# Raspy-Py/VolumetricRenderer

Measured on AMD Instinct MI355X. Metric: Mray/s (= W*H*steps/s) at 1080p x 128 steps, higher is better.
Workload: dtype f32; 1 GPU; grid512: 512^3 RGBA8 grid, 1920x1080, 128 steps, RGBA8 out; width=1920, height=1080, max_steps=128, volume=512^3 RGBA8, camera=reference (TestMain.cpp:219-245), kernel=grid_col48_clamp_uG

## Files before the change

volumetricrenderer_amd/csrc/vr_ctx.h:

```cpp
#pragma once

#include <algorithm>
#include <cmath>
#include <cstdarg>
#include <cstdio>
#include <cstring>
#include <exception>
#include <new>
#include <stdexcept>
#include <string>
#include <vector>

#include "../../include/vr.h"
#include "vr_internal.h"

namespace vrapi {
using namespace vr;

extern thread_local std::string g_err;
vr_status fail(vr_status st, const char* fmt, ...);
vr_status caught_exception(const char* fn) noexcept;

#define HIP_TRY(expr)                                                                        \
    do {                                                                                     \
// ... 132 lines not shown
    bool region_exact = false;
    long long renders_since_build = 0;
    std::vector<float> sort_key;
    long long renders_since_sort = 0;
    int sort_reuse = 0;
    int lattice = 1;
    int inject_throw = 0;
    unsigned long long gen = 1;
    int launch_cache = 1;
    int empty_fill = 1;
    int frames_overlap = 0;
    int row_setup = 40, row_pow = 130;
    int row_first_pct = 100;
    struct Cached {
        bool valid = false;
        unsigned long long gen = 0;
        vr_target t{};
        hipStream_t stream = nullptr;
        GridFrame f;
    } lc[4];
    int lc_next = 0;
    long long lc_hits = 0;
    int pair_deal = 0;
    int frame_pairing = 2;
    long long pair_launches = 0;
    int frame_group = 4;
    long long group_launches = 0;
    int frame_quad = 1;
    long long quad_launches = 0;
    int quad_split = 1;
    long long quad_split_launches = 0;
    int quad_steps = 1;
    long long quad_steps_launches = 0;
    uint2* d_lat = nullptr;
    size_t lat_cap = 0;
    long long lat_key[3] = {0, 0, -1};
};

constexpr long long kMaxWorleyTableBytes = 32 << 10;

int auto_layout(int nx, int ny, int nz);
Ctx* as_ctx(void* p);
void free_volume(Ctx* c);
bool dims_ok(int nx, int ny, int nz);
int wanted_fast_layout(const Ctx* c);
vr_status ensure_fast_layout(Ctx* c, hipStream_t s);
vr_status install_volume(Ctx* c, const uint8_t* d_rgba, int nx, int ny, int nz, hipStream_t s);
vr_status resolve_uniform(Ctx* c);
vr_status ensure_blur(Ctx* c, size_t need);
vr_status release_blur(Ctx* c);
void tap_constants(const Ctx* c, float S[4][3], float T[4][3]);
bool clamp_is_exact(const Ctx* c, const float S[4][3], const float T[4][3]);
int band_rows_packed(int height, int band_rows, int band_stride, int band_first, int band_flip = 0);
vr_status make_plan(Ctx* c, MarchArgs* a, Plan* p);
bool frame_args(const Ctx* c, int width, int height, MarchArgs* a);
inline float acc_limit_of(float transmittance, float density, float step_size)
{
    return transmittance > 0.0f ? (float)(-std::log((double)transmittance) / ((double)density * (double)step_size))
                                : INFINITY;
}
void proc_args(const Ctx* c, MarchArgs* a);
void volume_args(const Ctx* c, const Plan& pl, MarchArgs* a);
const char* variant_name(const Plan& p);

struct TargetInfo {
    int format;
// ... 33 lines not shown
```

volumetricrenderer_amd/csrc/vr_internal.h:

```cpp
#pragma once
#include <hip/hip_runtime.h>
#include <stdint.h>
#include <stddef.h>
#include "../../include/vr.h"
#include "vr_dispatch.h"

namespace vr {

enum Layout : int {
    LAYOUT_PLANAR = 1,
    LAYOUT_BRICK5 = 2,
    LAYOUT_BRICK8 = 3,
    LAYOUT_BRICK16 = 4,
    LAYOUT_CORNER8 = 5,
    LAYOUT_BRICK4 = 6,
    LAYOUT_ZPAIR = 7,
    LAYOUT_BRICK448 = 8,
    LAYOUT_BRICK488 = 9,
    LAYOUT_BRICK4816 = 10,
    LAYOUT_BRICK41616 = 11,
    LAYOUT_BRICK4832 = 12,
    LAYOUT_BRICK4864 = 13,
    LAYOUT_CORNERH = 14,
    LAYOUT_COL48 = 15,
// ... 135 lines not shown
    void* out;
    long long pitch;
    int format;
    int empty_fill;
    int bands_in_place;
    unsigned long long* step_counter;
    ProcParams proc;
    int slab_cap;
};

template <int L>
constexpr size_t march_lds_bytes(const MarchArgs& a)
{
    if (L == LAYOUT_PLANAR || L == LAYOUT_CORNERH) return 0;
    return (size_t)(a.nx + a.ny + a.nz + 3) * sizeof(unsigned) * (L == LAYOUT_COL48Z ? 2 : 1);
}

constexpr bool has_u_kernels(int l)
{
    return l == LAYOUT_COL48 || l == LAYOUT_BRICK4832 || l == LAYOUT_CORNERH || l == LAYOUT_COL48Z;
}
constexpr int u_kernel_channel(bool early, bool zero_offsets, int umask)
{
    if (early || !zero_offsets) return -1;
    return umask == 1 ? 0 : umask == 2 ? 1 : umask == 4 ? 2 : umask == 8 ? 3 : -1;
}

constexpr bool quad_instance(int layout, bool early, bool zero_offsets, int umask)
{
    if (u_kernel_channel(early, zero_offsets, umask) >= 0) return true;
    return !(is_b4_family(layout) && !early && zero_offsets);
}

enum QuadMode : int { QUAD_NONE = 0, QUAD_FRAMES = 1, QUAD_SPLIT = 2, QUAD_STEPS = 3 };
constexpr bool quad_split_layout(int layout) { return layout == LAYOUT_COL48 || layout == LAYOUT_BRICK4832; }

template <bool EARLY>
__host__ __device__ inline float quad_round_accumulate(float acc, float t0, float t1, float t2, float t3, int base, int n,
                                                       float acc_limit, bool* stop)
{
    bool st = false;
    const float t[4] = {t0, t1, t2, t3};
    for (int j = 0; j < 4; ++j) {
        acc = base + j < n && !st ? acc + t[j] : acc;
        if (EARLY) st = acc > acc_limit;
    }
    *stop = st;
    return acc;
}

struct FrameArgs {
    float org[3], o[3], px[3], py[3];
    float r2[4], r3[4];
    int cam_mode;
    float cam[3];
    float tap_T[4][3];
    int empty_fill;
    void* out;
    unsigned long long* step_counter;
};
__host__ __device__ inline FrameArgs frame_part(const MarchArgs& a)
{
    FrameArgs f{};
    for (int i = 0; i < 3; ++i) { f.org[i] = a.org[i]; f.o[i] = a.o[i]; f.px[i] = a.px[i]; f.py[i] = a.py[i]; f.cam[i] = a.cam[i]; }
    for (int i = 0; i < 4; ++i) { f.r2[i] = a.r2[i]; f.r3[i] = a.r3[i]; }
    for (int t = 0; t < 4; ++t)
        for (int i = 0; i < 3; ++i) f.tap_T[t][i] = a.tap_T[t][i];
    f.cam_mode = a.cam_mode;
// ... 308 lines not shown
```

volumetricrenderer_amd/csrc/vr_march_kernels.h:

```cpp
#pragma once
#include "vr_march_common.h"
#include "vr_noise.h"

namespace vr {
namespace {

constexpr int kTile = 16;

__device__ __forceinline__ float lerp_(float a, float b, float t) { return fmaf(t, b - a, a); }
__device__ __forceinline__ f2 lerp2(f2 a, f2 b, f2 t) { return __builtin_elementwise_fma(t, b - a, a); }
__device__ __forceinline__ int clampi(int v, int lo, int hi) { return min(max(v, lo), hi); }

__device__ __forceinline__ int cvt_flr(float x)
{
    int r;
    asm("v_cvt_flr_i32_f32 %0, %1" : "=v"(r) : "v"(x));
    return r;
}
__device__ __forceinline__ float fract_(float x) { return __builtin_amdgcn_fractf(x); }

template <int K>
__device__ __forceinline__ float ubyte(unsigned v)
{
    float r;
// ... 244 lines not shown
        float t0, t1, t2, t3;
        if constexpr (LAYOUT != LAYOUT_PLANAR) {
            t0 = blend_u<UM, 0, LAYOUT>(fetch_u<UM, 0, LAYOUT, ZO>(a, f, pxy, pz), uv);
            t1 = blend_u<UM, 1, LAYOUT>(fetch_u<UM, 1, LAYOUT, ZO>(a, f, pxy, pz), uv);
            t2 = blend_u<UM, 2, LAYOUT>(fetch_u<UM, 2, LAYOUT, ZO>(a, f, pxy, pz), uv);
            t3 = blend_u<UM, 3, LAYOUT>(fetch_u<UM, 3, LAYOUT, ZO>(a, f, pxy, pz), uv);
        } else {
            t0 = tap<LAYOUT, WRAP>(a, f, 0, pxy, pz);
            t1 = tap<LAYOUT, WRAP>(a, f, 1, pxy, pz);
            t2 = tap<LAYOUT, WRAP>(a, f, 2, pxy, pz);
            t3 = tap<LAYOUT, WRAP>(a, f, 3, pxy, pz);
        }
        acc = acc + ((t0 * t1) * (t2 + t3)) * (LAYOUT == LAYOUT_CORNERH ? f.scale : a.scale);
        pxy = pxy + r.sxy;
        pz = pz + r.sz;
        if constexpr (EARLY) {
            if (acc > a.acc_limit) { ++i; break; }
        }
    }
    if (r.live) {
        const float at = acc * a.step_size;
        store_pixel(a, x, orow, r.n >= 0, 1.0f - spec_expf(a.density * fminf(-at, 0.0f)));
    }
    return r.n > 0 ? (unsigned)i : 0u;
}

template <int J>
__device__ __forceinline__ unsigned quad_lane(unsigned v)
{
    return (unsigned)__builtin_amdgcn_update_dpp(0, (int)v, J * 0x55, 0xf, 0xf, true);
}
template <int K>
__device__ __forceinline__ float ubyte_of(unsigned v) { return (float)((v >> (8 * K)) & 0xffu); }

constexpr unsigned kSplitZ = 32;

struct SliceRaw {
    unsigned s0, s1, off;
};
template <int UM, int T, bool ZO>
__device__ __forceinline__ SliceRaw split_fetch(const MarchArgs& a, const FastCtx& f, f2 pxy, float pz, unsigned zoff)
{
    if constexpr ((UM >> T) & 1) {
        return SliceRaw{};
    } else {
        const f2 Tt = ZO ? f2{0.5f, 0.5f} : f2{a.tap_T[T][0], a.tap_T[T][1]};
        const f2 gxy = __builtin_elementwise_fma(pxy, f2{a.tap_S[T][0], a.tap_S[T][1]}, Tt);
        const float gz = fmaf(pz, a.tap_S[T][2], ZO ? 0.5f : a.tap_T[T][2]);
        const unsigned off = f.tx[cvt_flr(gxy.x)] + f.ty[cvt_flr(gxy.y)] + f.tz[cvt_flr(gz)];
        const auto s = __builtin_amdgcn_raw_buffer_load_b64(f.rsrc[T], (off & ~3u) + zoff, 0, 0);
        return SliceRaw{s[0], s[1], off};
    }
}
__device__ __forceinline__ unsigned split_pack(const SliceRaw& r)
{
    const unsigned q0 = __builtin_amdgcn_alignbyte(r.s1, r.s0, r.off);
    const unsigned q1 = __builtin_amdgcn_alignbyte(r.s1, r.s1, r.off);
    return __builtin_amdgcn_perm(q1, q0, 0x05040100u);
}
template <int UM, int T, int H, bool ZO>
__device__ __forceinline__ float split_blend(const MarchArgs& a, unsigned pk, f2 pxy, float pz, const float* uv)
{
    if constexpr ((UM >> T) & 1) {
        return uv[T];
    } else {
        const f2 Tt = ZO ? f2{0.5f, 0.5f} : f2{a.tap_T[T][0], a.tap_T[T][1]};
        const f2 gxy = __builtin_elementwise_fma(pxy, f2{a.tap_S[T][0], a.tap_S[T][1]}, Tt);
        const float gz = fmaf(pz, a.tap_S[T][2], ZO ? 0.5f : a.tap_T[T][2]);
// ... 34 lines not shown
            const unsigned p0 = split_pack(c0), p1 = split_pack(c1), p2 = split_pack(c2), p3 = split_pack(c3);
            bool stop = false;
            {
                const float t0 = split_blend<UM, 0, 0, ZO>(a, p0, axy, az, uv), t1 = split_blend<UM, 1, 0, ZO>(a, p1, axy, az, uv);
                const float t2 = split_blend<UM, 2, 0, ZO>(a, p2, axy, az, uv), t3 = split_blend<UM, 3, 0, ZO>(a, p3, axy, az, uv);
                acc = acc + ((t0 * t1) * (t2 + t3)) * a.scale;
                if constexpr (EARLY) stop = acc > a.acc_limit;
            }
            __builtin_amdgcn_sched_barrier(0);
            {
                const float t0 = split_blend<UM, 0, 1, ZO>(a, p0, bxy, bz, uv), t1 = split_blend<UM, 1, 1, ZO>(a, p1, bxy, bz, uv);
                const float t2 = split_blend<UM, 2, 1, ZO>(a, p2, bxy, bz, uv), t3 = split_blend<UM, 3, 1, ZO>(a, p3, bxy, bz, uv);
                const float both = acc + ((t0 * t1) * (t2 + t3)) * a.scale;
                acc = i + 1 < r.n && !stop ? both : acc;
                if constexpr (EARLY) stop = acc > a.acc_limit;
            }
            i += 2;
            if (stop || i >= r.n) break;
            c0 = n0; c1 = n1; c2 = n2; c3 = n3;
            axy = cxy; az = cz;
            bxy = dxy; bz = dz;
        }
    }
    if (r.live) {
        const float at = acc * a.step_size;
        store_pixel(a, x, orow, r.n >= 0, 1.0f - spec_expf(a.density * fminf(-at, 0.0f)));
    }
}

struct StepRaw {
    unsigned s00, s01, s10, s11, off;
    float wx, wy, wz;
};
template <int UM, int T, bool ZO>
__device__ __forceinline__ StepRaw step_fetch(const MarchArgs& a, const FastCtx& f, f2 pxy, float pz)
{
    if constexpr ((UM >> T) & 1) {
        return StepRaw{};
    } else {
        const f2 Tt = ZO ? f2{0.5f, 0.5f} : f2{a.tap_T[T][0], a.tap_T[T][1]};
        const f2 gxy = __builtin_elementwise_fma(pxy, f2{a.tap_S[T][0], a.tap_S[T][1]}, Tt);
        const float gz = fmaf(pz, a.tap_S[T][2], ZO ? 0.5f : a.tap_T[T][2]);
        const unsigned off = f.tx[cvt_flr(gxy.x)] + f.ty[cvt_flr(gxy.y)] + f.tz[cvt_flr(gz)];
        const auto s0 = __builtin_amdgcn_raw_buffer_load_b64(f.rsrc[T], off & ~3u, 0, 0);
        const auto s1 = __builtin_amdgcn_raw_buffer_load_b64(f.rsrc[T], (off & ~3u) + kSplitZ, 0, 0);
        return StepRaw{s0[0], s0[1], s1[0], s1[1], off, fract_(gxy.x), fract_(gxy.y), fract_(gz)};
    }
}
__device__ __forceinline__ TapRaw step_tap(const StepRaw& r)
{
    return TapRaw{__builtin_amdgcn_alignbyte(r.s01, r.s00, r.off), __builtin_amdgcn_alignbyte(r.s01, r.s01, r.off),
                  __builtin_amdgcn_alignbyte(r.s11, r.s10, r.off), __builtin_amdgcn_alignbyte(r.s11, r.s11, r.off),
                  r.wx, r.wy, r.wz};
}
template <int J>
__device__ __forceinline__ float quad_lane_f(float v)
{
    return __builtin_bit_cast(float, quad_lane<J>(__builtin_bit_cast(unsigned, v)));
}
template <int LAYOUT, bool EARLY, bool ZO, int UM>
__device__ __forceinline__ void march_pixel_quad_steps(const MarchArgs& a, const FastCtx& f, int x, int orow, int fl)
{
    static_assert(quad_split_layout(LAYOUT), "built for the layouts of the split fetch");
    const Ray r = setup_ray(a, x, orow);
    float uv[4] = {};
    if constexpr (UM != 0)
        for (int t = 0; t < 4; ++t)
            if ((UM >> t) & 1) uv[t] = noise::in_vgpr(a.uval[t]);
    float acc = 0.0f;
    if (r.n > 0) {
        const auto own = [fl](auto p0, auto p1, auto p2, auto p3) { return fl & 2 ? (fl & 1 ? p3 : p2) : (fl & 1 ? p1 : p0); };
        f2 axy = r.pxy;
        float az = r.pz;
        f2 bxy = axy + r.sxy, cxy = bxy + r.sxy, dxy = cxy + r.sxy;
        float bz = az + r.sz, cz = bz + r.sz, dz = cz + r.sz;
        bool mine = fl < r.n;
        f2 qxy = mine ? own(axy, bxy, cxy, dxy) : axy;
        float qz = mine ? own(az, bz, cz, dz) : az;
        StepRaw c0 = step_fetch<UM, 0, ZO>(a, f, qxy, qz), c1 = step_fetch<UM, 1, ZO>(a, f, qxy, qz);
        StepRaw c2 = step_fetch<UM, 2, ZO>(a, f, qxy, qz), c3 = step_fetch<UM, 3, ZO>(a, f, qxy, qz);
        for (int base = 0;;) {
            const f2 exy = dxy + r.sxy, fxy = exy + r.sxy, gxy = fxy + r.sxy, hxy = gxy + r.sxy;
            const float ez = dz + r.sz, fz = ez + r.sz, gz = fz + r.sz, hz = gz + r.sz;
            mine = base + 4 + fl < r.n;
            qxy = mine ? own(exy, fxy, gxy, hxy) : axy;
            qz = mine ? own(ez, fz, gz, hz) : az;
            const StepRaw n0 = step_fetch<UM, 0, ZO>(a, f, qxy, qz), n1 = step_fetch<UM, 1, ZO>(a, f, qxy, qz);
            const StepRaw n2 = step_fetch<UM, 2, ZO>(a, f, qxy, qz), n3 = step_fetch<UM, 3, ZO>(a, f, qxy, qz);
            const float t0 = blend_u<UM, 0, LAYOUT>(step_tap(c0), uv), t1 = blend_u<UM, 1, LAYOUT>(step_tap(c1), uv);
            const float t2 = blend_u<UM, 2, LAYOUT>(step_tap(c2), uv), t3 = blend_u<UM, 3, LAYOUT>(step_tap(c3), uv);
            const float term = ((t0 * t1) * (t2 + t3)) * a.scale;
            __builtin_amdgcn_sched_barrier(0);
            bool stop;
            acc = quad_round_accumulate<EARLY>(acc, quad_lane_f<0>(term), quad_lane_f<1>(term), quad_lane_f<2>(term),
                                               quad_lane_f<3>(term), base, r.n, a.acc_limit, &stop);
            base += 4;
            if (stop || base >= r.n) break;
            c0 = n0; c1 = n1; c2 = n2; c3 = n3;
            axy = exy; az = ez;
            dxy = hxy; dz = hz;
        }
    }
    if (r.live) {
        const float at = acc * a.step_size;
        store_pixel(a, x, orow, r.n >= 0, 1.0f - spec_expf(a.density * fminf(-at, 0.0f)));
    }
}

template <int LAYOUT>
__device__ __forceinline__ FastCtx fast_prologue(const MarchArgs& a, unsigned* lds)
{
    FastCtx f{};
    if constexpr (LAYOUT == LAYOUT_CORNERH) {
        for (int c = 0; c < 4; ++c)
            f.rsrc[c] = __builtin_amdgcn_make_buffer_rsrc((void*)(a.vol + (size_t)c * a.plane_stride), (short)0,
                                                          (int)a.plane_stride, 0x00020000);
        f.s1x16 = (float)(16 * a.geom.nbx);
        f.s2x16 = (float)(16 * a.geom.nbx) * (float)a.geom.nby;
        for (int c = 0; c < 4; ++c) {
            f.sz[c] = noise::in_vgpr(a.tap_S[c][2]);
            f.oz[c] = noise::in_vgpr(a.tap_T[c][2]);
        }
        f.scale = noise::in_vgpr(a.scale);
// ... 111 lines not shown
    if ((int)(blockIdx.x >> 3) * WGW >= count) return;
#ifdef VR_TIMELINE
    const unsigned long long t_begin = __builtin_amdgcn_s_memrealtime();
#endif
    const FastCtx f = fast_prologue<LAYOUT>(a, lds);
    const int lane = threadIdx.x & 63;
    unsigned long long steps = 0;
    for (int k = w; w < nwx && k < count; k += nwx) {
        const unsigned t = tiles[begin + k];
        const int tx = (int)(t & 0xffffu), ty = (int)(t >> 16);
        steps += march_pixel<LAYOUT, WRAP, EARLY, ZO, UM>(a, f, tx * 8 + lane_x<LAYOUT>(lane),
                                                          ty * 8 + lane_y<LAYOUT>(lane));
    }
#ifdef VR_TIMELINE
    timeline_record(t_begin, steps);
#endif
    if (a.step_counter) add_steps(a, steps);
}
template <int LAYOUT, int WRAP, bool EARLY, bool ZO, int WGW = kThreads / 64>
__global__ __launch_bounds__(64 * WGW) void march_regions(const MarchArgs a, const unsigned* __restrict__ tiles,
                                                         const int* __restrict__ hdr, int nwx)
{
    extern __shared__ __attribute__((aligned(16))) unsigned lds[];
    regions_body<LAYOUT, WRAP, EARLY, ZO, WGW, 0>(a, tiles, hdr, nwx, lds);
}
template <int LAYOUT, int WRAP, bool EARLY, bool ZO, int UM>
__global__ __launch_bounds__(kThreads) void march_regions_u(const MarchArgs a, const unsigned* __restrict__ tiles,
                                                           const int* __restrict__ hdr, int nwx)
{
    extern __shared__ __attribute__((aligned(16))) unsigned lds[];
    regions_body<LAYOUT, WRAP, EARLY, ZO, kThreads / 64, UM>(a, tiles, hdr, nwx, lds);
}

template <int LAYOUT, int WRAP, bool EARLY, bool ZO, int UM, int NF, bool QUAD = false, bool SPLIT = false, bool STEPS = false>
__device__ __forceinline__ void regions_frames_body(const FramesArgs<NF>& g, const unsigned* __restrict__ tiles,
                                                    const int* __restrict__ hdr, int nwx, int deal, unsigned* lds)
{
    static_assert(NF == 2 || NF == 4, "a 4-wave workgroup is 4 / NF entry waves x NF frames");
    static_assert(!QUAD || NF == 4, "a quad of lanes is four frames");
    static_assert(!SPLIT || QUAD, "the lanes of a quad split a fetch only where they hold one ray");
    static_assert(!STEPS || SPLIT, "the step rounds are a split launch's");
    const int xcd = blockIdx.x & 7, wg = (int)(blockIdx.x >> 3);
    const int wave = __builtin_amdgcn_readfirstlane((int)(threadIdx.x >> 6));
    int fr = wave, first = wg, w = wg;
    if constexpr (NF == 2) {
        fr = deal ? (wg & 1) : (wave & 1);
        first = deal ? (wg >> 1) * 4 : wg * 2;
        w = first + (deal ? wave : (wave >> 1));
    }
    const int begin = hdr[xcd], all = hdr[xcd + 1] - begin;
    const int marched = min(hdr[kRegionWork + xcd], all);
    MarchArgs a = g.c;
    set_frame(&a, g.fr[fr]);
    const int count = a.empty_fill ? marched : all;
    if (a.empty_fill) fill_empty_tiles(a, tiles, begin, count, all, w, nwx);
    bool every = g.fr[0].empty_fill;
    for (int k = 1; k < NF; ++k) every = every && g.fr[k].empty_fill;
    if (first >= (every ? marched : all)) return;
    FastCtx f = fast_prologue<LAYOUT>(g.c, lds);
    const int lane = threadIdx.x & 63;
    if constexpr (QUAD) {
        MarchArgs q = g.c;
        const int fl = lane & 3;
        void* out = g.fr[0].out;
        for (int k = 1; k < NF; ++k) out = fl == k ? g.fr[k].out : out;
        q.out = out;
        const int qx = (wave & 1) * 4 + ((lane >> 2) & 3), qy = (wave >> 1) * 4 + (lane >> 4);
        const int qcount = g.c.empty_fill ? marched : all;
        for (int k = wg; wg < nwx && k < qcount; k += nwx) {
            const unsigned t = tiles[begin + k];
            const int tx = (int)(t & 0xffffu), ty = (int)(t >> 16);
            if constexpr (STEPS) march_pixel_quad_steps<LAYOUT, EARLY, ZO, UM>(q, f, tx * 8 + qx, ty * 8 + qy, fl);
            else if constexpr (SPLIT) march_pixel_quad_split<LAYOUT, EARLY, ZO, UM>(q, f, tx * 8 + qx, ty * 8 + qy, fl);
            else (void)march_pixel<LAYOUT, WRAP, EARLY, ZO, UM>(q, f, tx * 8 + qx, ty * 8 + qy);
        }
        return;
    }
    if constexpr (LAYOUT == LAYOUT_CORNERH)
        for (int c = 0; c < 4; ++c) f.oz[c] = noise::in_vgpr(a.tap_T[c][2]);
    unsigned long long steps = 0;
    for (int k = w; w < nwx && k < count; k += nwx) {
        const unsigned t = tiles[begin + k];
        const int tx = (int)(t & 0xffffu), ty = (int)(t >> 16);
        steps += march_pixel<LAYOUT, WRAP, EARLY, ZO, UM>(a, f, tx * 8 + lane_x<LAYOUT>(lane),
                                                          ty * 8 + lane_y<LAYOUT>(lane));
    }
    if (a.step_counter) add_steps(a, steps);
}
#define VR_SPLIT_WAVES __attribute__((amdgpu_waves_per_eu(SPLIT && (!STEPS || ZO) ? 5 : 1)))
template <int LAYOUT, int WRAP, bool EARLY, bool ZO, int NF, bool QUAD = false, bool SPLIT = false, bool STEPS = false>
__global__ __launch_bounds__(kThreads) VR_SPLIT_WAVES void march_regions_frames(const FramesArgs<NF> g, const unsigned* __restrict__ tiles,
                                                                const int* __restrict__ hdr, int nwx, int deal)
{
    extern __shared__ __attribute__((aligned(16))) unsigned lds[];
    regions_frames_body<LAYOUT, WRAP, EARLY, ZO, 0, NF, QUAD, SPLIT, STEPS>(g, tiles, hdr, nwx, deal, lds);
}
template <int LAYOUT, int WRAP, bool EARLY, bool ZO, int UM, int NF, bool QUAD = false, bool SPLIT = false, bool STEPS = false>
__global__ __launch_bounds__(kThreads) VR_SPLIT_WAVES void march_regions_frames_u(const FramesArgs<NF> g, const unsigned* __restrict__ tiles,
                                                                  const int* __restrict__ hdr, int nwx, int deal)
{
    extern __shared__ __attribute__((aligned(16))) unsigned lds[];
    regions_frames_body<LAYOUT, WRAP, EARLY, ZO, UM, NF, QUAD, SPLIT, STEPS>(g, tiles, hdr, nwx, deal, lds);
}
#undef VR_SPLIT_WAVES


template <int LAYOUT, bool EARLY, bool ZO, int K, int UM = 0>
__device__ __forceinline__ unsigned march_pixel_split(const MarchArgs& a, const FastCtx& f, int x, int orow,
                                                      int k, int ray_lane)
{
    constexpr int R = 64 / K;
    const Ray r = setup_ray(a, x, orow);
    float uv[4] = {};
    if constexpr (UM != 0)
        for (int t = 0; t < 4; ++t)
            if ((UM >> t) & 1) uv[t] = noise::in_vgpr(a.uval[t]);
    const int n = r.n;
    f2 pxy = r.pxy;
    float pz = r.pz;
    for (int j = 0; j < k; ++j) { pxy = pxy + r.sxy; pz = pz + r.sz; }
    float acc = 0.0f;
    int i = 0;
    if (n > 0) {
        const bool mine0 = k < n;
        TapRaw c0 = fetch_u<UM, 0, LAYOUT, ZO>(a, f, mine0 ? pxy : r.pxy, mine0 ? pz : r.pz);
        TapRaw c1 = fetch_u<UM, 1, LAYOUT, ZO>(a, f, mine0 ? pxy : r.pxy, mine0 ? pz : r.pz);
        TapRaw c2 = fetch_u<UM, 2, LAYOUT, ZO>(a, f, mine0 ? pxy : r.pxy, mine0 ? pz : r.pz);
        TapRaw c3 = fetch_u<UM, 3, LAYOUT, ZO>(a, f, mine0 ? pxy : r.pxy, mine0 ? pz : r.pz);
        for (int base = 0; base < n; base += K) {
            for (int j = 0; j < K; ++j) { pxy = pxy + r.sxy; pz = pz + r.sz; }
            const bool mine = base + K + k < n;
            const f2 qxy = mine ? pxy : r.pxy;
            const float qz = mine ? pz : r.pz;
            const TapRaw n0 = fetch_u<UM, 0, LAYOUT, ZO>(a, f, qxy, qz), n1 = fetch_u<UM, 1, LAYOUT, ZO>(a, f, qxy, qz);
            const TapRaw n2 = fetch_u<UM, 2, LAYOUT, ZO>(a, f, qxy, qz), n3 = fetch_u<UM, 3, LAYOUT, ZO>(a, f, qxy, qz);
// ... 180 lines not shown
    if (sc.kind == SCHED_REGIONS) return regions(std::integral_constant<int, 4>{});
#if VR_EXPERIMENTS
    if (sc.kind == SCHED_XCDROWS) {
        const int groups = (((a.width + 7) >> 3) + 3) >> 2, rows8 = (a.out_rows + 7) >> 3;
        const dim3 grid(8 * ((rows8 + 7) / 8) * groups);
        return with_bool(early, [&](auto E) {
            hipLaunchKernelGGL((march_xcdrows<L, W, E>), grid, block, lds, s, a);
            return hipGetLastError();
        });
    }
    if (sc.kind == SCHED_QUEUE) {
        hipError_t e = hipMemsetAsync(sc.heads, 0, 32, s);
        if (e != hipSuccess) return e;
        const dim3 grid(256 * sc.waves_per_simd);
        return with_bool(early, [&](auto E) {
            hipLaunchKernelGGL((march_queue<L, W, E>), grid, block, lds, s, a, sc.heads);
            return hipGetLastError();
        });
    }
#endif
    const dim3 grid(a.num_blocks);
    return with_bool(early, [&](auto E) {
        hipLaunchKernelGGL((march_grid<L, W, E>), grid, block, lds, s, a);
        return hipGetLastError();
    });
}

template <int L, int W>
hipError_t launch_frames_l(const MarchArgs& a, const FrameArgs* fr, int nf, bool early, const Schedule& sc, int deal, int quad,
                           hipStream_t s)
{
    if (quad != QUAD_NONE && (nf != kGroupFrames || !quad_instance(L, early, a.zero_offsets != 0, a.umask)))
        return hipErrorInvalidValue;
    if ((quad == QUAD_SPLIT || quad == QUAD_STEPS) && !quad_split_layout(L)) return hipErrorInvalidValue;
    return with_value<2, kGroupFrames>(nf, [&](auto NF) { return with_value<QUAD_NONE, QUAD_FRAMES, QUAD_SPLIT, QUAD_STEPS>(quad, [&](auto QD) {
        constexpr bool Q = decltype(QD)::value != QUAD_NONE && decltype(NF)::value == kGroupFrames;
        constexpr bool ST = Q && decltype(QD)::value == QUAD_STEPS && quad_split_layout(L);
        constexpr bool SP = (Q && decltype(QD)::value == QUAD_SPLIT && quad_split_layout(L)) || ST;
        FramesArgs<NF> g;
        g.c = a;
        for (int k = 0; k < NF; ++k) g.fr[k] = fr[k];
        const size_t lds = march_lds_bytes<L>(a);
        const dim3 block(kThreads);
        static_assert(has_u_kernels(L), "every multi-frame layout has the _u kernels");
        static_assert(kThreads == 64 * 4, "a workgroup is 4 / NF entry waves x NF frames");
        const int nwx = sc.map.nwx;
        const int dl = NF == 4 ? 0 : deal;
        const dim3 grid((unsigned)(NF == 4 ? 8 * nwx : dl ? 16 * ((nwx + 3) / 4) : 8 * ((nwx + 1) / 2)));
        if (u_kernel_channel(early, a.zero_offsets, a.umask) >= 0)
            return with_value<1, 2, 4, 8>(a.umask, [&](auto U) {
                hipLaunchKernelGGL((march_regions_frames_u<L, W, false, true, U, NF, Q, SP, ST>), grid, block, lds, s, g, sc.tiles, sc.hdr, nwx, dl);
                return hipGetLastError();
            }, hipErrorInvalidValue);
        return with_bool(early, [&](auto E) { return with_bool(a.zero_offsets, [&](auto Z) {
            constexpr bool QG = Q && quad_instance(L, decltype(E)::value, decltype(Z)::value, 0);
            hipLaunchKernelGGL((march_regions_frames<L, W, E, Z, NF, QG, QG && SP, QG && ST>), grid, block, lds, s, g, sc.tiles, sc.hdr, nwx, dl);
            return hipGetLastError();
        }); });
    }, hipErrorInvalidValue); }, hipErrorInvalidValue);
}

}
}
```

volumetricrenderer_amd/csrc/vr_options.cpp:

```cpp
#include "vr_ctx.h"

using namespace vrapi;

extern "C" {

vr_status vr_set_layout_preference(void* p, int pref)
try {
    if (!p || pref < 0 || pref >= kNumLayouts) return fail(VR_ERR_INVALID, "vr_set_layout_preference: bad argument");
    if (pref > 0 && !layout_built(pref))
        return fail(VR_ERR_INVALID, "vr_set_layout_preference: layout %d is built only with VR_EXPERIMENTS "
                                    "(make EXPERIMENTS=1; measured slower, DESIGN.md sec. 4)", pref);
    Ctx* c = as_ctx(p);
    ++c->gen;
    HIP_TRY(hipSetDevice(c->device));
    c->layout_pref = pref;
    vr_status st = ensure_fast_layout(c, nullptr);
    if (st == VR_OK && hipDeviceSynchronize() != hipSuccess) return fail(VR_ERR_HIP, "vr_set_layout_preference: sync");
    return st;
} catch (...) {
    return caught_exception("vr_set_layout_preference");
}

vr_status vr_set_option(void* p, const char* name, int value)
try {
// ... 32 lines not shown
        if (value < 0 || value > 1) return fail(VR_ERR_INVALID, "vr_set_option: empty_fill is 0 or 1");
        c->empty_fill = value;
        ++c->gen;
        return VR_OK;
    }
    if (n == "frame_pairing") {
        if (value < 0 || value > 2) return fail(VR_ERR_INVALID, "vr_set_option: frame_pairing is 0, 1 or 2");
        c->frame_pairing = value;
        return VR_OK;
    }
    if (n == "frame_group") {
        if (value != 2 && value != 4) return fail(VR_ERR_INVALID, "vr_set_option: frame_group is 2 or 4");
        c->frame_group = value;
        return VR_OK;
    }
    if (n == "pair_deal") {
        if (value < 0 || value > 1) return fail(VR_ERR_INVALID, "vr_set_option: pair_deal is 0 or 1");
        c->pair_deal = value;
        return VR_OK;
    }
    if (n == "frame_quad") {
        if (value < 0 || value > 1) return fail(VR_ERR_INVALID, "vr_set_option: frame_quad is 0 or 1");
        c->frame_quad = value;
        return VR_OK;
    }
    if (n == "quad_split") {
        if (value < 0 || value > 1) return fail(VR_ERR_INVALID, "vr_set_option: quad_split is 0 or 1");
        c->quad_split = value;
        return VR_OK;
    }
    if (n == "quad_steps") {
        if (value < 0 || value > 1) return fail(VR_ERR_INVALID, "vr_set_option: quad_steps is 0 or 1");
        c->quad_steps = value;
        return VR_OK;
    }
    if (n == "inject_throw") {
        if (value < 0 || value > 2)
            return fail(VR_ERR_INVALID, "vr_set_option: inject_throw is 0, 1 (std::runtime_error) or 2 (std::bad_alloc)");
        c->inject_throw = value;
        return VR_OK;
    }
    if (n == "schedule") {
        if (value < -1 || value > 5)
            return fail(VR_ERR_INVALID, "vr_set_option: schedule is -1 (auto), 0 (static), 1 (queue), "
                                        "2 (strided), 3 (xcd rows), 4 (rings) or 5 (regions)");
        c->schedule = value;
        return VR_OK;
    }
    if (n == "waves_per_simd") {
        if (value < 1 || value > 8) return fail(VR_ERR_INVALID, "vr_set_option: waves_per_simd in [1, 8]");
        c->waves_per_simd = value;
        return VR_OK;
    }
    if (n == "tiles_per_wave") {
        if (value < 0 || value > 64)
            return fail(VR_ERR_INVALID, "vr_set_option: tiles_per_wave in [1, 64], or 0 for auto");
        c->tiles_per_wave = value;
        return VR_OK;
    }
    if (n == "split") {
        if (value != 0 && value != 1 && value != 2 && value != 4 && value != 8)
            return fail(VR_ERR_INVALID, "vr_set_option: split is 0 (auto), 1, 2, 4 or 8");
        c->split = value;
        return VR_OK;
    }
    if (n == "wedges") {
// ... 131 lines not shown
    if (n == "blur_scratch_kib") return (int)std::min<size_t>(c->blur_bytes / 1024, 0x7fffffff);
    if (n == "slab_cap") return c->slab_cap;
    if (n == "region_order") return c->region_order;
    if (n == "sort_reuse") return c->sort_reuse;
    if (n == "wg_waves") return c->wg_waves;
    if (n == "uniform_skip") return c->uniform_skip;
    if (n == "region_work_tiles")
        return c->region_cur >= 0 ? c->region[c->region_cur].nwork : -1;
    if (n == "region_empty_tiles") {
        poll_region_header(c);
        return c->region_cur >= 0 ? c->region[c->region_cur].nempty : -1;
    }
    if (n == "uniform_mask") {
        if (!c->d_planar || resolve_uniform(c) != VR_OK) return -1;
        return c->uniform_mask;
    }
    if (n == "supertile") return c->supertile;
    if (n == "launch_cache") return c->launch_cache;
    if (n == "empty_fill") return c->empty_fill;
    if (n == "frames_overlap") return c->frames_overlap;
    if (n == "row_setup") return c->row_setup;
    if (n == "row_pow") return c->row_pow;
    if (n == "row_first_pct") return c->row_first_pct;
    if (n == "frame_pairing") return c->frame_pairing;
    if (n == "pair_deal") return c->pair_deal;
    if (n == "frame_group") return c->frame_group;
    if (n == "group_launches") return (int)std::min<long long>(c->group_launches, 0x7fffffff);
    if (n == "pair_launches") return (int)std::min<long long>(c->pair_launches, 0x7fffffff);
    if (n == "frame_quad") return c->frame_quad;
    if (n == "quad_split") return c->quad_split;
    if (n == "quad_split_launches") return (int)std::min<long long>(c->quad_split_launches, 0x7fffffff);
    if (n == "quad_steps") return c->quad_steps;
    if (n == "quad_steps_launches") return (int)std::min<long long>(c->quad_steps_launches, 0x7fffffff);
    if (n == "quad_launches") return (int)std::min<long long>(c->quad_launches, 0x7fffffff);
    if (n == "launch_cache_hits") return (int)std::min<long long>(c->lc_hits, 0x7fffffff);
    if (n == "experiments") return VR_EXPERIMENTS;
    if (n == "region_interval") return c->region_interval;
    if (n == "region_gpu") return c->region_gpu;
    if (n == "region_gpu_builds") return (int)std::min<long long>(c->gpu_builds, 0x7fffffff);
    return -1;
} catch (...) {
    (void)caught_exception("vr_get_option");
    return -1;
}

const char* vr_kernel_variant(void* p)
try {
    if (!p) return "none";
    Ctx* c = as_ctx(p);
    if (c->proc.enabled) {
        if (c->schedule == SCHED_STATIC) return c->proc.shadow_steps > 0 ? "procedural_shadow_tiles" : "procedural_tiles";
        if (c->schedule == SCHED_RINGS) return c->proc.shadow_steps > 0 ? "procedural_shadow_rings" : "procedural_rings";
        return c->proc.shadow_steps > 0 ? "procedural_shadow" : "procedural";
    }
    if (!c->d_planar || !c->has_camera) return "none";
    if (resolve_uniform(c) != VR_OK) return "none";
    MarchArgs a{};
    Plan pl{};
    make_plan(c, &a, &pl);
    const int kind = c->schedule >= 0 ? c->schedule : SCHED_REGIONS;
    if (pl.layout == LAYOUT_COL48 && c->slab && kind == SCHED_REGIONS && c->split <= 1)
        return pl.early ? "grid_col48_slab_clamp_early" : "grid_col48_slab_clamp";
    const int um = c->uniform_skip ? c->uniform_mask : 0;
    int ch = -1;
    if (kind == SCHED_REGIONS && c->wg_waves == 4 && has_u_kernels(pl.layout))
        ch = u_kernel_channel(pl.early, a.zero_offsets, um);
// ... 23 lines not shown
```

volumetricrenderer_amd/csrc/vr_render.cpp:

```cpp
#include "vr_ctx.h"

namespace vrapi {

vr_status check_frame_state(const char* fn, const Ctx* c, const vr_target* t)
{
    if (!c->d_planar && !c->proc.enabled)
        return fail(VR_ERR_NO_VOLUME, "%s: no volume (vr_set_volume / vr_generate_volume)", fn);
    if (!c->has_camera) return fail(VR_ERR_NO_CAMERA, "%s: no shader data (vr_set_shader_data)", fn);
    if (t->width <= 0 || t->height <= 0) return fail(VR_ERR_INVALID, "%s: bad size %dx%d", fn, t->width, t->height);
    return VR_OK;
}

vr_status check_pixels(const char* fn, const vr_target* t, int format, size_t* pitch)
{
    if (!t->pixels) return fail(VR_ERR_INVALID, "%s: pixels is null", fn);
    const int bpp = format_bytes(format);
    *pitch = t->row_pitch ? t->row_pitch : (size_t)t->width * bpp;
    if (*pitch < (size_t)t->width * bpp || *pitch % bpp != 0 || ((uintptr_t)t->pixels % bpp) != 0)
        return fail(VR_ERR_INVALID, "%s: pitch/alignment (pitch %zu, bpp %d)", fn, *pitch, bpp);
    return VR_OK;
}

vr_status check_target(const char* fn, const Ctx* c, const vr_target* t, TargetInfo* ti)
{
// ... 270 lines not shown
    bool grouped = groupable;
    for (int k = 1; k < n && groupable; ++k) {
        if (osd) st = vr_set_shader_data(p, &osd[k], &gsd[k]);
        if (st == VR_OK) st = grid_frame_args(c, &t[k], ti, &f[k]);
        if (st != VR_OK) {
            const std::string msg = g_err;
            vr_status rs = frame0_alone();
            if (rs == VR_OK) rs = render_plain(p, t, 1, k, osd, gsd, stream);
            if (osd) (void)vr_set_shader_data(p, &osd[k], &gsd[k]);
            g_err = msg;
            return st;
        }
        grouped = grouped && f[k].kind == f[0].kind && pair_compatible(f[0], f[k]);
    }
    if (!grouped) {
        st = frame0_alone();
        return st == VR_OK ? render_plain(p, t, 1, n, osd, gsd, stream) : st;
    }
    const Ctx::RegionBuf& rb = c->region[c->region_cur];
    FrameArgs fr[VR_MAX_GROUP];
    bool every = f[0].a.empty_fill != 0;
    for (int k = 0; k < n; ++k) {
        if (k > 0) f[k].a.empty_fill = f[0].a.empty_fill && same_region_camera(f[0], f[k]) ? 1 : 0;
        every = every && f[k].a.empty_fill;
        fr[k] = frame_part(f[k].a);
    }
    Schedule sc = f[0].sc;
    if (f[0].a.empty_fill && !every) sc.map.nwx = std::max(1, rb.map.nwx);
    bool quad = c->frame_quad && frames_share_camera(fr, n) &&
                quad_instance(f[0].pl.layout, f[0].pl.early, f[0].a.zero_offsets != 0, f[0].a.umask);
    for (int k = 0; k < n; ++k) quad = quad && !fr[k].step_counter;
    const bool split = quad && c->quad_split && quad_split_layout(f[0].pl.layout);
    const bool steps = split && c->quad_steps;
    HIP_TRY(launch_march_frames(f[0].a, fr, n, f[0].pl.layout, f[0].pl.early, sc, c->pair_deal,
                                steps ? QUAD_STEPS : split ? QUAD_SPLIT : quad ? QUAD_FRAMES : QUAD_NONE, hs));
    c->quad_launches += quad;
    c->quad_split_launches += split;
    c->quad_steps_launches += steps;
    c->group_launches += n == VR_MAX_GROUP;
    c->pair_launches += n / 2;
    c->renders_since_build += n - 1;
    c->region_slot = f[0].slot;
    return note_region_render(c, hs);
}

}

extern "C" {

vr_status vr_render(void* p, const vr_target* t, void* stream)
try {
    if (!p || !t) return fail(VR_ERR_INVALID, "vr_render: null argument");
    Ctx* c = as_ctx(p);
    TargetInfo ti;
    if (const vr_status st = check_target("vr_render", c, t, &ti)) return st;
    honour_inject_throw(c);
    const hipStream_t hs = static_cast<hipStream_t>(stream);
    if (c->proc.enabled) return render_procedural_frame(c, t, ti, hs);
    const GridFrame* hit = nullptr;
    if (const vr_status st = cache_hit(c, t, hs, &hit)) return st;
    if (hit) return launch_frame(c, *hit, nullptr, 0, hs);
    GridFrame f;
    if (const vr_status st = grid_frame_args(c, t, ti, &f)) return st;
    if (f.kind == SCHED_REGIONS)
        if (const vr_status st = attach_regions(c, hs, &f)) return st;
    return launch_frame(c, f, t, c->gen, hs);
} catch (...) {
    return caught_exception("vr_render");
}

vr_status vr_render_sequence(void* p, const vr_target* t, int frames, const vr_object_shader_data* osd,
// ... 61 lines not shown
```

Baseline: 6.205 million Mray/s.

## Pair z-slice fetches across quad lanes with DPP exchange in step rounds

```diff
diff --git a/volumetricrenderer_amd/csrc/vr_ctx.h b/volumetricrenderer_amd/csrc/vr_ctx.h
--- a/volumetricrenderer_amd/csrc/vr_ctx.h
+++ b/volumetricrenderer_amd/csrc/vr_ctx.h
@@ -188,6 +188,8 @@
     long long quad_split_launches = 0;
     int quad_steps = 1;
     long long quad_steps_launches = 0;
+    int quad_pairs = 1;
+    long long quad_pairs_launches = 0;
     uint2* d_lat = nullptr;
     size_t lat_cap = 0;
     long long lat_key[3] = {0, 0, -1};
diff --git a/volumetricrenderer_amd/csrc/vr_internal.h b/volumetricrenderer_amd/csrc/vr_internal.h
--- a/volumetricrenderer_amd/csrc/vr_internal.h
+++ b/volumetricrenderer_amd/csrc/vr_internal.h
@@ -191,8 +191,25 @@
     return !(is_b4_family(layout) && !early && zero_offsets);
 }
 
-enum QuadMode : int { QUAD_NONE = 0, QUAD_FRAMES = 1, QUAD_SPLIT = 2, QUAD_STEPS = 3 };
+enum QuadMode : int { QUAD_NONE = 0, QUAD_FRAMES = 1, QUAD_SPLIT = 2, QUAD_STEPS = 3, QUAD_PAIRS = 4 };
 constexpr bool quad_split_layout(int layout) { return layout == LAYOUT_COL48 || layout == LAYOUT_BRICK4832; }
+constexpr unsigned kSplitZ = 32;
+
+constexpr __host__ __device__ int pair_load_step(int instr, int fl) { return 2 * instr + (fl >> 1); }
+constexpr __host__ __device__ int pair_load_slice(int fl) { return fl & 1; }
+constexpr __host__ __device__ int pair_owner_instr(int j) { return j >> 1; }
+constexpr __host__ __device__ int pair_owner_lane(int j, int z) { return 2 * (j & 1) + z; }
+constexpr __host__ __device__ int quad_perm_ctrl(int l0, int l1, int l2, int l3) { return l0 | l1 << 2 | l2 << 4 | l3 << 6; }
+constexpr __host__ __device__ int pair_load_ctrl(int instr)
+{
+    return quad_perm_ctrl(pair_load_step(instr, 0), pair_load_step(instr, 1), pair_load_step(instr, 2), pair_load_step(instr, 3));
+}
+constexpr __host__ __device__ int pair_owner_ctrl(int z)
+{
+    return quad_perm_ctrl(pair_owner_lane(0, z), pair_owner_lane(1, z), pair_owner_lane(2, z), pair_owner_lane(3, z));
+}
+static_assert(pair_load_ctrl(0) == 0x50 && pair_load_ctrl(1) == 0xfa, "quad_perm [0,0,1,1] and [2,2,3,3]");
+static_assert(pair_owner_ctrl(0) == 0x88 && pair_owner_ctrl(1) == 0xdd, "quad_perm [0,2,0,2] and [1,3,1,3]");
 
 template <bool EARLY>
 __host__ __device__ inline float quad_round_accumulate(float acc, float t0, float t1, float t2, float t3, int base, int n,
diff --git a/volumetricrenderer_amd/csrc/vr_march_kernels.h b/volumetricrenderer_amd/csrc/vr_march_kernels.h
--- a/volumetricrenderer_amd/csrc/vr_march_kernels.h
+++ b/volumetricrenderer_amd/csrc/vr_march_kernels.h
@@ -300,8 +300,6 @@
 }
 template <int K>
 __device__ __forceinline__ float ubyte_of(unsigned v) { return (float)((v >> (8 * K)) & 0xffu); }
-
-constexpr unsigned kSplitZ = 32;
 
 struct SliceRaw {
     unsigned s0, s1, off;
@@ -402,8 +400,18 @@
     unsigned s00, s01, s10, s11, off;
     float wx, wy, wz;
 };
-template <int UM, int T, bool ZO>
-__device__ __forceinline__ StepRaw step_fetch(const MarchArgs& a, const FastCtx& f, f2 pxy, float pz)
+template <int J>
+__device__ __forceinline__ float quad_lane_f(float v)
+{
+    return __builtin_bit_cast(float, quad_lane<J>(__builtin_bit_cast(unsigned, v)));
+}
+template <int CTRL>
+__device__ __forceinline__ unsigned quad_read(unsigned v)
+{
+    return (unsigned)__builtin_amdgcn_update_dpp(0, (int)v, CTRL, 0xf, 0xf, true);
+}
+template <int UM, int T, bool ZO, bool PAIRS = false>
+__device__ __forceinline__ StepRaw step_fetch(const MarchArgs& a, const FastCtx& f, f2 pxy, float pz, int fl = 0)
 {
     if constexpr ((UM >> T) & 1) {
         return StepRaw{};
@@ -412,9 +420,18 @@
         const f2 gxy = __builtin_elementwise_fma(pxy, f2{a.tap_S[T][0], a.tap_S[T][1]}, Tt);
         const float gz = fmaf(pz, a.tap_S[T][2], ZO ? 0.5f : a.tap_T[T][2]);
         const unsigned off = f.tx[cvt_flr(gxy.x)] + f.ty[cvt_flr(gxy.y)] + f.tz[cvt_flr(gz)];
-        const auto s0 = __builtin_amdgcn_raw_buffer_load_b64(f.rsrc[T], off & ~3u, 0, 0);
-        const auto s1 = __builtin_amdgcn_raw_buffer_load_b64(f.rsrc[T], (off & ~3u) + kSplitZ, 0, 0);
-        return StepRaw{s0[0], s0[1], s1[0], s1[1], off, fract_(gxy.x), fract_(gxy.y), fract_(gz)};
+        if constexpr (PAIRS) {
+            const unsigned zoff = (unsigned)pair_load_slice(fl) * kSplitZ;
+            const unsigned al = off & ~3u;
+            const auto sa = __builtin_amdgcn_raw_buffer_load_b64(f.rsrc[T], quad_read<pair_load_ctrl(0)>(al) + zoff, 0, 0);
+            const auto sb = __builtin_amdgcn_raw_buffer_load_b64(f.rsrc[T], quad_read<pair_load_ctrl(1)>(al) + zoff, 0, 0);
+            const unsigned sh = (quad_read<pair_load_ctrl(0)>(off) & 3u) | (quad_read<pair_load_ctrl(1)>(off) << 2);
+            return StepRaw{sa[0], sa[1], sb[0], sb[1], sh, fract_(gxy.x), fract_(gxy.y), fract_(gz)};
+        } else {
+            const auto s0 = __builtin_amdgcn_raw_buffer_load_b64(f.rsrc[T], off & ~3u, 0, 0);
+            const auto s1 = __builtin_amdgcn_raw_buffer_load_b64(f.rsrc[T], (off & ~3u) + kSplitZ, 0, 0);
+            return StepRaw{s0[0], s0[1], s1[0], s1[1], off, fract_(gxy.x), fract_(gxy.y), fract_(gz)};
+        }
     }
 }
 __device__ __forceinline__ TapRaw step_tap(const StepRaw& r)
@@ -423,12 +440,23 @@
                   __builtin_amdgcn_alignbyte(r.s11, r.s10, r.off), __builtin_amdgcn_alignbyte(r.s11, r.s11, r.off),
                   r.wx, r.wy, r.wz};
 }
-template <int J>
-__device__ __forceinline__ float quad_lane_f(float v)
-{
-    return __builtin_bit_cast(float, quad_lane<J>(__builtin_bit_cast(unsigned, v)));
-}
-template <int LAYOUT, bool EARLY, bool ZO, int UM>
+template <int UM, int T>
+__device__ __forceinline__ float pair_blend(const StepRaw& r, int fl, const float* uv)
+{
+    if constexpr ((UM >> T) & 1) {
+        return uv[T];
+    } else {
+        const unsigned pa = split_pack(SliceRaw{r.s00, r.s01, r.off}), pb = split_pack(SliceRaw{r.s10, r.s11, r.off >> 2});
+        const unsigned a0 = quad_read<pair_owner_ctrl(0)>(pa), b0 = quad_read<pair_owner_ctrl(0)>(pb);
+        const unsigned a1 = quad_read<pair_owner_ctrl(1)>(pa), b1 = quad_read<pair_owner_ctrl(1)>(pb);
+        const bool second = pair_owner_instr(fl) != 0;
+        const unsigned z0 = second ? b0 : a0, z1 = second ? b1 : a1;
+        return blend(f2{ubyte_of<0>(z0), ubyte_of<0>(z1)}, f2{ubyte_of<1>(z0), ubyte_of<1>(z1)},
+                     f2{ubyte_of<2>(z0), ubyte_of<2>(z1)}, f2{ubyte_of<3>(z0), ubyte_of<3>(z1)}, r.wx, r.wy, r.wz);
+    }
+}
+
+template <int LAYOUT, bool EARLY, bool ZO, int UM, bool PAIRS = false>
 __device__ __forceinline__ void march_pixel_quad_steps(const MarchArgs& a, const FastCtx& f, int x, int orow, int fl)
 {
     static_assert(quad_split_layout(LAYOUT), "built for the layouts of the split fetch");
@@ -447,18 +475,20 @@
         bool mine = fl < r.n;
         f2 qxy = mine ? own(axy, bxy, cxy, dxy) : axy;
         float qz = mine ? own(az, bz, cz, dz) : az;
-        StepRaw c0 = step_fetch<UM, 0, ZO>(a, f, qxy, qz), c1 = step_fetch<UM, 1, ZO>(a, f, qxy, qz);
-        StepRaw c2 = step_fetch<UM, 2, ZO>(a, f, qxy, qz), c3 = step_fetch<UM, 3, ZO>(a, f, qxy, qz);
+        StepRaw c0 = step_fetch<UM, 0, ZO, PAIRS>(a, f, qxy, qz, fl), c1 = step_fetch<UM, 1, ZO, PAIRS>(a, f, qxy, qz, fl);
+        StepRaw c2 = step_fetch<UM, 2, ZO, PAIRS>(a, f, qxy, qz, fl), c3 = step_fetch<UM, 3, ZO, PAIRS>(a, f, qxy, qz, fl);
         for (int base = 0;;) {
             const f2 exy = dxy + r.sxy, fxy = exy + r.sxy, gxy = fxy + r.sxy, hxy = gxy + r.sxy;
             const float ez = dz + r.sz, fz = ez + r.sz, gz = fz + r.sz, hz = gz + r.sz;
             mine = base + 4 + fl < r.n;
             qxy = mine ? own(exy, fxy, gxy, hxy) : axy;
             qz = mine ? own(ez, fz, gz, hz) : az;
-            const StepRaw n0 = step_fetch<UM, 0, ZO>(a, f, qxy, qz), n1 = step_fetch<UM, 1, ZO>(a, f, qxy, qz);
-            const StepRaw n2 = step_fetch<UM, 2, ZO>(a, f, qxy, qz), n3 = step_fetch<UM, 3, ZO>(a, f, qxy, qz);
-            const float t0 = blend_u<UM, 0, LAYOUT>(step_tap(c0), uv), t1 = blend_u<UM, 1, LAYOUT>(step_tap(c1), uv);
-            const float t2 = blend_u<UM, 2, LAYOUT>(step_tap(c2), uv), t3 = blend_u<UM, 3, LAYOUT>(step_tap(c3), uv);
+            const StepRaw n0 = step_fetch<UM, 0, ZO, PAIRS>(a, f, qxy, qz, fl), n1 = step_fetch<UM, 1, ZO, PAIRS>(a, f, qxy, qz, fl);
+            const StepRaw n2 = step_fetch<UM, 2, ZO, PAIRS>(a, f, qxy, qz, fl), n3 = step_fetch<UM, 3, ZO, PAIRS>(a, f, qxy, qz, fl);
+            const float t0 = PAIRS ? pair_blend<UM, 0>(c0, fl, uv) : blend_u<UM, 0, LAYOUT>(step_tap(c0), uv);
+            const float t1 = PAIRS ? pair_blend<UM, 1>(c1, fl, uv) : blend_u<UM, 1, LAYOUT>(step_tap(c1), uv);
+            const float t2 = PAIRS ? pair_blend<UM, 2>(c2, fl, uv) : blend_u<UM, 2, LAYOUT>(step_tap(c2), uv);
+            const float t3 = PAIRS ? pair_blend<UM, 3>(c3, fl, uv) : blend_u<UM, 3, LAYOUT>(step_tap(c3), uv);
             const float term = ((t0 * t1) * (t2 + t3)) * a.scale;
             __builtin_amdgcn_sched_barrier(0);
             bool stop;
@@ -636,7 +666,8 @@
     regions_body<LAYOUT, WRAP, EARLY, ZO, kThreads / 64, UM>(a, tiles, hdr, nwx, lds);
 }
 
-template <int LAYOUT, int WRAP, bool EARLY, bool ZO, int UM, int NF, bool QUAD = false, bool SPLIT = false, bool STEPS = false>
+template <int LAYOUT, int WRAP, bool EARLY, bool ZO, int UM, int NF, bool QUAD = false, bool SPLIT = false, bool STEPS = false,
+          bool PAIRS = false>
 __device__ __forceinline__ void regions_frames_body(const FramesArgs<NF>& g, const unsigned* __restrict__ tiles,
                                                     const int* __restrict__ hdr, int nwx, int deal, unsigned* lds)
 {
@@ -644,6 +675,7 @@
     static_assert(!QUAD || NF == 4, "a quad of lanes is four frames");
     static_assert(!SPLIT || QUAD, "the lanes of a quad split a fetch only where they hold one ray");
     static_assert(!STEPS || SPLIT, "the step rounds are a split launch's");
+    static_assert(!PAIRS || STEPS, "the paired fetch is the step rounds'");
     const int xcd = blockIdx.x & 7, wg = (int)(blockIdx.x >> 3);
     const int wave = __builtin_amdgcn_readfirstlane((int)(threadIdx.x >> 6));
     int fr = wave, first = wg, w = wg;
@@ -674,7 +706,7 @@
         for (int k = wg; wg < nwx && k < qcount; k += nwx) {
             const unsigned t = tiles[begin + k];
             const int tx = (int)(t & 0xffffu), ty = (int)(t >> 16);
-            if constexpr (STEPS) march_pixel_quad_steps<LAYOUT, EARLY, ZO, UM>(q, f, tx * 8 + qx, ty * 8 + qy, fl);
+            if constexpr (STEPS) march_pixel_quad_steps<LAYOUT, EARLY, ZO, UM, PAIRS>(q, f, tx * 8 + qx, ty * 8 + qy, fl);
             else if constexpr (SPLIT) march_pixel_quad_split<LAYOUT, EARLY, ZO, UM>(q, f, tx * 8 + qx, ty * 8 + qy, fl);
             else (void)march_pixel<LAYOUT, WRAP, EARLY, ZO, UM>(q, f, tx * 8 + qx, ty * 8 + qy);
         }
@@ -691,20 +723,21 @@
     }
     if (a.step_counter) add_steps(a, steps);
 }
-#define VR_SPLIT_WAVES __attribute__((amdgpu_waves_per_eu(SPLIT && (!STEPS || ZO) ? 5 : 1)))
-template <int LAYOUT, int WRAP, bool EARLY, bool ZO, int NF, bool QUAD = false, bool SPLIT = false, bool STEPS = false>
-__global__ __launch_bounds__(kThreads) VR_SPLIT_WAVES void march_regions_frames(const FramesArgs<NF> g, const unsigned* __restrict__ tiles,
+#define VR_SPLIT_WAVES(E) __attribute__((amdgpu_waves_per_eu(SPLIT && (!STEPS || ZO) && !(PAIRS && (E)) ? 5 : 1)))
+template <int LAYOUT, int WRAP, bool EARLY, bool ZO, int NF, bool QUAD = false, bool SPLIT = false, bool STEPS = false, bool PAIRS = false>
+__global__ __launch_bounds__(kThreads) VR_SPLIT_WAVES(EARLY) void march_regions_frames(const FramesArgs<NF> g, const unsigned* __restrict__ tiles,
                                                                 const int* __restrict__ hdr, int nwx, int deal)
 {
     extern __shared__ __attribute__((aligned(16))) unsigned lds[];
-    regions_frames_body<LAYOUT, WRAP, EARLY, ZO, 0, NF, QUAD, SPLIT, STEPS>(g, tiles, hdr, nwx, deal, lds);
-}
-template <int LAYOUT, int WRAP, bool EARLY, bool ZO, int UM, int NF, bool QUAD = false, bool SPLIT = false, bool STEPS = false>
-__global__ __launch_bounds__(kThreads) VR_SPLIT_WAVES void march_regions_frames_u(const FramesArgs<NF> g, const unsigned* __restrict__ tiles,
+    regions_frames_body<LAYOUT, WRAP, EARLY, ZO, 0, NF, QUAD, SPLIT, STEPS, PAIRS>(g, tiles, hdr, nwx, deal, lds);
+}
+template <int LAYOUT, int WRAP, bool EARLY, bool ZO, int UM, int NF, bool QUAD = false, bool SPLIT = false, bool STEPS = false,
+          bool PAIRS = false>
+__global__ __launch_bounds__(kThreads) VR_SPLIT_WAVES(false) void march_regions_frames_u(const FramesArgs<NF> g, const unsigned* __restrict__ tiles,
                                                                   const int* __restrict__ hdr, int nwx, int deal)
 {
     extern __shared__ __attribute__((aligned(16))) unsigned lds[];
-    regions_frames_body<LAYOUT, WRAP, EARLY, ZO, UM, NF, QUAD, SPLIT, STEPS>(g, tiles, hdr, nwx, deal, lds);
+    regions_frames_body<LAYOUT, WRAP, EARLY, ZO, UM, NF, QUAD, SPLIT, STEPS, PAIRS>(g, tiles, hdr, nwx, deal, lds);
 }
 #undef VR_SPLIT_WAVES
 
@@ -951,10 +984,11 @@
 {
     if (quad != QUAD_NONE && (nf != kGroupFrames || !quad_instance(L, early, a.zero_offsets != 0, a.umask)))
         return hipErrorInvalidValue;
-    if ((quad == QUAD_SPLIT || quad == QUAD_STEPS) && !quad_split_layout(L)) return hipErrorInvalidValue;
-    return with_value<2, kGroupFrames>(nf, [&](auto NF) { return with_value<QUAD_NONE, QUAD_FRAMES, QUAD_SPLIT, QUAD_STEPS>(quad, [&](auto QD) {
+    if ((quad == QUAD_SPLIT || quad == QUAD_STEPS || quad == QUAD_PAIRS) && !quad_split_layout(L)) return hipErrorInvalidValue;
+    return with_value<2, kGroupFrames>(nf, [&](auto NF) { return with_value<QUAD_NONE, QUAD_FRAMES, QUAD_SPLIT, QUAD_STEPS, QUAD_PAIRS>(quad, [&](auto QD) {
         constexpr bool Q = decltype(QD)::value != QUAD_NONE && decltype(NF)::value == kGroupFrames;
-        constexpr bool ST = Q && decltype(QD)::value == QUAD_STEPS && quad_split_layout(L);
+        constexpr bool PR = Q && decltype(QD)::value == QUAD_PAIRS && quad_split_layout(L);
+        constexpr bool ST = (Q && decltype(QD)::value == QUAD_STEPS && quad_split_layout(L)) || PR;
         constexpr bool SP = (Q && decltype(QD)::value == QUAD_SPLIT && quad_split_layout(L)) || ST;
         FramesArgs<NF> g;
         g.c = a;
@@ -968,12 +1002,12 @@
         const dim3 grid((unsigned)(NF == 4 ? 8 * nwx : dl ? 16 * ((nwx + 3) / 4) : 8 * ((nwx + 1) / 2)));
         if (u_kernel_channel(early, a.zero_offsets, a.umask) >= 0)
             return with_value<1, 2, 4, 8>(a.umask, [&](auto U) {
-                hipLaunchKernelGGL((march_regions_frames_u<L, W, false, true, U, NF, Q, SP, ST>), grid, block, lds, s, g, sc.tiles, sc.hdr, nwx, dl);
+                hipLaunchKernelGGL((march_regions_frames_u<L, W, false, true, U, NF, Q, SP, ST, PR>), grid, block, lds, s, g, sc.tiles, sc.hdr, nwx, dl);
                 return hipGetLastError();
             }, hipErrorInvalidValue);
         return with_bool(early, [&](auto E) { return with_bool(a.zero_offsets, [&](auto Z) {
             constexpr bool QG = Q && quad_instance(L, decltype(E)::value, decltype(Z)::value, 0);
-            hipLaunchKernelGGL((march_regions_frames<L, W, E, Z, NF, QG, QG && SP, QG && ST>), grid, block, lds, s, g, sc.tiles, sc.hdr, nwx, dl);
+            hipLaunchKernelGGL((march_regions_frames<L, W, E, Z, NF, QG, QG && SP, QG && ST, QG && PR>), grid, block, lds, s, g, sc.tiles, sc.hdr, nwx, dl);
             return hipGetLastError();
         }); });
     }, hipErrorInvalidValue); }, hipErrorInvalidValue);
diff --git a/volumetricrenderer_amd/csrc/vr_options.cpp b/volumetricrenderer_amd/csrc/vr_options.cpp
--- a/volumetricrenderer_amd/csrc/vr_options.cpp
+++ b/volumetricrenderer_amd/csrc/vr_options.cpp
@@ -88,6 +88,11 @@
     if (n == "quad_steps") {
         if (value < 0 || value > 1) return fail(VR_ERR_INVALID, "vr_set_option: quad_steps is 0 or 1");
         c->quad_steps = value;
+        return VR_OK;
+    }
+    if (n == "quad_pairs") {
+        if (value < 0 || value > 1) return fail(VR_ERR_INVALID, "vr_set_option: quad_pairs is 0 or 1");
+        c->quad_pairs = value;
         return VR_OK;
     }
     if (n == "inject_throw") {
@@ -285,6 +290,8 @@
     if (n == "quad_split_launches") return (int)std::min<long long>(c->quad_split_launches, 0x7fffffff);
     if (n == "quad_steps") return c->quad_steps;
     if (n == "quad_steps_launches") return (int)std::min<long long>(c->quad_steps_launches, 0x7fffffff);
+    if (n == "quad_pairs") return c->quad_pairs;
+    if (n == "quad_pairs_launches") return (int)std::min<long long>(c->quad_pairs_launches, 0x7fffffff);
     if (n == "quad_launches") return (int)std::min<long long>(c->quad_launches, 0x7fffffff);
     if (n == "launch_cache_hits") return (int)std::min<long long>(c->lc_hits, 0x7fffffff);
     if (n == "experiments") return VR_EXPERIMENTS;
diff --git a/volumetricrenderer_amd/csrc/vr_render.cpp b/volumetricrenderer_amd/csrc/vr_render.cpp
--- a/volumetricrenderer_amd/csrc/vr_render.cpp
+++ b/volumetricrenderer_amd/csrc/vr_render.cpp
@@ -326,11 +326,13 @@
     for (int k = 0; k < n; ++k) quad = quad && !fr[k].step_counter;
     const bool split = quad && c->quad_split && quad_split_layout(f[0].pl.layout);
     const bool steps = split && c->quad_steps;
+    const bool pairs = steps && c->quad_pairs;
     HIP_TRY(launch_march_frames(f[0].a, fr, n, f[0].pl.layout, f[0].pl.early, sc, c->pair_deal,
-                                steps ? QUAD_STEPS : split ? QUAD_SPLIT : quad ? QUAD_FRAMES : QUAD_NONE, hs));
+                                pairs ? QUAD_PAIRS : steps ? QUAD_STEPS : split ? QUAD_SPLIT : quad ? QUAD_FRAMES : QUAD_NONE, hs));
     c->quad_launches += quad;
     c->quad_split_launches += split;
     c->quad_steps_launches += steps;
+    c->quad_pairs_launches += pairs;
     c->group_launches += n == VR_MAX_GROUP;
     c->pair_launches += n / 2;
     c->renders_since_build += n - 1;
```

Measured after the change: 6.633 million Mray/s (median of 6 runs). 6.9% higher.
